# zifuwan/Sigma

Measured on AMD Instinct MI355X. Metric: images/sec fwd+bwd sigma_small 480x640, higher is better.
Workload: dtype f32

## Files before the change

include/sigma_ops.h:

```cpp
#ifndef SIGMA_OPS_H_
#define SIGMA_OPS_H_

#include <stdint.h>

#ifdef __cplusplus
extern "C" {
#endif

enum sigma_ops_status {
    SIGMA_OPS_OK = 0,
    SIGMA_OPS_ERR_ARG = 1,
    SIGMA_OPS_ERR_LAUNCH = 5
};

typedef struct sigma_dwconv_params {
    int32_t batch, channels, height, width;
    int32_t n_orders;
    int32_t flags;
    const float *x;
    const float *weight;
    const float *bias;
    float *out2;
    const float *g2;
    float *gpre;
// ... 14 lines not shown
typedef struct sigma_merge_params {
    int32_t batch, channels, height, width;
    const float *planes4;
    float *planes2;
    float *nhwc;
} sigma_merge_params;

int sigma_cross_merge_nhwc(const sigma_merge_params *params, void *stream);
int sigma_cross_split_nhwc(const sigma_merge_params *params, void *stream);

typedef struct sigma_transpose_params {
    int32_t batch, rows, cols, reserved_;
    const float *src;
    float *dst;
    int64_t src_batch_stride, src_row_stride, dst_batch_stride, dst_row_stride;
} sigma_transpose_params;

int sigma_transpose2d(const sigma_transpose_params *params, void *stream);

int sigma_pair_sum_add(const float *src, float *acc, int64_t n_outer, int64_t inner, void *stream);

int sigma_upsample2x_nhwc(const float *in, float *out, int32_t batch, int32_t height, int32_t width, int32_t channels,
                          int32_t backward, void *stream);

int sigma_plane_pool(const float *x, int64_t planes, int64_t hw, float *mean, float *max, float *count, void *stream);
int sigma_plane_scale(const float *x, const float *scale, float *out, int64_t planes, int64_t hw, void *stream);
int sigma_plane_dot(const float *a, const float *b, float *out, int64_t planes, int64_t hw, void *stream);
typedef struct sigma_gate_bwd_params {
    int64_t planes, hw;
    const float *g;
    const float *x;
    const float *scale;
    const float *dmean;
    const float *dmax;
    const float *max;
    const float *count;
    float *dx;
} sigma_gate_bwd_params;
int sigma_plane_gate_bwd(const sigma_gate_bwd_params *params, void *stream);

#define SIGMA_CE_BLOCKS 1024
int sigma_softmax_ce_fwd(const float *logits, const int64_t *labels, int64_t rows, int32_t classes, int64_t ignore_index,
                         float *lse, float *partial, void *stream);
int sigma_softmax_ce_bwd(const float *logits, const int64_t *labels, const float *lse, const float *scale, int64_t rows,
                         int32_t classes, int64_t ignore_index, float *dlogits, void *stream);
int sigma_softmax_ce_fwd_ld(const float *logits, const int64_t *labels, int64_t rows, int32_t classes, int32_t ld,
// ... 155 lines not shown
```

sigma_amd/_capi.py:

```python
from __future__ import annotations

import ctypes
import os
from typing import Optional

_HERE = os.path.dirname(os.path.abspath(__file__))
LIB_PATH = os.environ.get("SIGMA_HIP_LIB") or os.path.join(_HERE, "lib", "libsigma_hip.so")

SIGMA_SCAN_ABI_VERSION = 13
SIGMA_SCAN_CHUNK = 2048
SIGMA_SCAN_CKPT_PITCH = 1280
SIGMA_SCAN_CKPT_PITCH_FINE = 640
SIGMA_SCAN_CKPT_PITCH_320 = 320
SIGMA_SCAN_CKPT_PITCH_160 = 160
SIGMA_SCAN_CKPT_PITCH_16 = 16
SIGMA_SCAN_MAX_DSTATE = 256
SIGMA_SCAN_BWD_DETERMINISTIC = 1
SIGMA_DWCONV_DETERMINISTIC = 1

DTYPE_F32, DTYPE_F16, DTYPE_BF16 = 0, 1, 2


class SigmaHipUnavailable(RuntimeError):
    pass
# ... 60 lines not shown
class TransposeParams(ctypes.Structure):
    _fields_ = [
        ("batch", ctypes.c_int32), ("rows", ctypes.c_int32), ("cols", ctypes.c_int32), ("reserved_", ctypes.c_int32),
        ("src", ctypes.c_void_p), ("dst", ctypes.c_void_p),
        ("src_batch_stride", ctypes.c_int64), ("src_row_stride", ctypes.c_int64),
        ("dst_batch_stride", ctypes.c_int64), ("dst_row_stride", ctypes.c_int64),
    ]


class LayerNormParams(ctypes.Structure):
    _fields_ = [
        ("rows", ctypes.c_int64), ("channels", ctypes.c_int32), ("eps", ctypes.c_float),
        ("x", ctypes.c_void_p), ("gamma", ctypes.c_void_p), ("beta", ctypes.c_void_p),
        ("y", ctypes.c_void_p), ("mean", ctypes.c_void_p), ("rstd", ctypes.c_void_p),
        ("dy", ctypes.c_void_p), ("dx", ctypes.c_void_p), ("dgamma", ctypes.c_void_p), ("dbeta", ctypes.c_void_p),
        ("workspace", ctypes.c_void_p),
        ("gate", ctypes.c_void_p), ("gate_row_stride", ctypes.c_int64), ("dgate", ctypes.c_void_p),
        ("dgate_row_stride", ctypes.c_int64),
        ("row_scale", ctypes.c_void_p), ("rows_per_scale", ctypes.c_int64),
        ("dx_add", ctypes.c_void_p),
    ]


class GemmParams(ctypes.Structure):
    _fields_ = [
        ("M", ctypes.c_int64), ("N", ctypes.c_int32), ("K", ctypes.c_int32),
        ("A", ctypes.c_void_p), ("Bt", ctypes.c_void_p), ("C", ctypes.c_void_p), ("bias", ctypes.c_void_p),
        ("lda", ctypes.c_int64), ("ldb", ctypes.c_int64), ("ldc", ctypes.c_int64),
        ("accumulate", ctypes.c_int32), ("batch", ctypes.c_int32),
        ("strideA", ctypes.c_int64), ("strideB", ctypes.c_int64), ("strideC", ctypes.c_int64),
        ("a_mod", ctypes.c_int32), ("pieces", ctypes.c_int32),
        ("c_mod", ctypes.c_int32), ("reserved", ctypes.c_int32),
        ("residual", ctypes.c_void_p), ("residual2", ctypes.c_void_p), ("ldr", ctypes.c_int64), ("strideR", ctypes.c_int64),
        ("Ct", ctypes.c_void_p), ("ldct", ctypes.c_int64), ("t_cols", ctypes.c_int32), ("k_slices", ctypes.c_int32),
        ("workspace", ctypes.c_void_p), ("workspace_bytes", ctypes.c_int64),
    ]


class GateBwdParams(ctypes.Structure):
    _fields_ = [
        ("planes", ctypes.c_int64), ("hw", ctypes.c_int64),
        ("g", ctypes.c_void_p), ("x", ctypes.c_void_p), ("scale", ctypes.c_void_p), ("dmean", ctypes.c_void_p),
        ("dmax", ctypes.c_void_p), ("max", ctypes.c_void_p), ("count", ctypes.c_void_p), ("dx", ctypes.c_void_p),
    ]


# ... 47 lines not shown
    _fields_ = [
        ("batch", ctypes.c_int32), ("height", ctypes.c_int32), ("width", ctypes.c_int32), ("scale", ctypes.c_int32),
        ("classes", ctypes.c_int32), ("ld", ctypes.c_int32), ("ignore_index", ctypes.c_int64),
        ("kind", ctypes.c_int32), ("label_smoothing", ctypes.c_float), ("gamma", ctypes.c_float), ("reserved_", ctypes.c_int32),
        ("logits", ctypes.c_void_p), ("labels", ctypes.c_void_p), ("weight", ctypes.c_void_p), ("lse", ctypes.c_void_p),
        ("row_loss", ctypes.c_void_p), ("coef", ctypes.c_void_p), ("partial", ctypes.c_void_p),
        ("scale_grad", ctypes.c_void_p), ("row_grad", ctypes.c_void_p), ("dlogits", ctypes.c_void_p),
    ]


SIGMA_CE_BLOCKS = 1024
SIGMA_UPSAMPLE_LOSS_OPTIONS, SIGMA_UPSAMPLE_LOSS_FOCAL = 0, 1
SIGMA_OHEM_HIST_BLOCKS = 512
SIGMA_SEG_LDS_HIST_BYTES = 32768

GEMM_FORMS = {"nt": 0, "nn": 1, "tn": 2}
GEMM_EPILOGUES = ("rows", "direct", "transposed")
GEMM_RES_LOADS = ("none", "vector", "scalar")
GEMM_STORES = ("store", "accumulate", "atomic")

STRUCTS = {
    "sigma_scan_fwd_params": FwdParams, "sigma_scan_bwd_params": BwdParams,
    "sigma_dwconv_params": DwConvParams, "sigma_merge_params": MergeParams, "sigma_transpose_params": TransposeParams,
    "sigma_layernorm_params": LayerNormParams, "sigma_gate_bwd_params": GateBwdParams,
    "sigma_seg_accumulate_params": SegAccumulateParams, "sigma_seg_confusion_params": SegConfusionParams,
    "sigma_ce_opt_params": CeOptParams, "sigma_ohem_params": OhemParams, "sigma_upsample_ce_params": UpsampleCeParams,
    "sigma_upsample_loss_params": UpsampleLossParams,
    "sigma_gemm_params": GemmParams,
}

_I32, _I64, _INT, _F32, _VP, _STR = (ctypes.c_int32, ctypes.c_int64, ctypes.c_int, ctypes.c_float, ctypes.c_void_p,
                                     ctypes.c_char_p)
_P = ctypes.POINTER


def _params_stream(struct, *names):
    return {n: (_INT, [_P(struct), _VP]) for n in names}


_SCAN_SIGNATURES = {
    **_params_stream(FwdParams, "sigma_selective_scan_fwd"),
    **_params_stream(BwdParams, "sigma_selective_scan_bwd"),
    "sigma_scan_bwd_workspace_bytes": (_I64, [_P(BwdParams)]),
    "sigma_scan_fwd_workspace_bytes": (_I64, [_P(FwdParams)]),
    "sigma_scan_last_error": (_STR, []),
    "sigma_scan_abi_version": (_INT, []),
    "sigma_scan_set_option": (_INT, [_STR, _INT]),
    "sigma_scan_get_option": (_INT, [_STR]),
    "sigma_scan_fwd_plan": (_INT, [_P(FwdParams), _P(_I32 * 6)]),
    "sigma_scan_bwd_plan": (_INT, [_P(BwdParams), _P(_I32 * 6)]),
    "sigma_scan_selftest": (_INT, [_VP]),
    "sigma_scan_rowlane_selftest": (_INT, [_VP]),
}
_OPS_SIGNATURES = {
    **_params_stream(DwConvParams, "sigma_dwconv3x3_silu_fwd", "sigma_dwconv3x3_silu_bwd"),
    **_params_stream(MergeParams, "sigma_cross_merge_nhwc", "sigma_cross_split_nhwc"),
    **_params_stream(LayerNormParams, "sigma_layernorm_fwd", "sigma_layernorm_bwd"),
    "sigma_layernorm_bwd_partial_rows": (_INT, [_I64, _I32]),
    **_params_stream(TransposeParams, "sigma_transpose2d"),
    "sigma_pair_sum_add": (_INT, [_VP, _VP, _I64, _I64, _VP]),
    "sigma_upsample2x_nhwc": (_INT, [_VP, _VP, _I32, _I32, _I32, _I32, _I32, _VP]),
    "sigma_plane_pool": (_INT, [_VP, _I64, _I64, _VP, _VP, _VP, _VP]),
    "sigma_plane_scale": (_INT, [_VP, _VP, _VP, _I64, _I64, _VP]),
    "sigma_plane_dot": (_INT, [_VP, _VP, _VP, _I64, _I64, _VP]),
    **_params_stream(GateBwdParams, "sigma_plane_gate_bwd"),
    "sigma_softmax_ce_fwd": (_INT, [_VP, _VP, _I64, _I32, _I64, _VP, _VP, _VP]),
    "sigma_softmax_ce_bwd": (_INT, [_VP, _VP, _VP, _VP, _I64, _I32, _I64, _VP, _VP]),
    "sigma_softmax_ce_fwd_ld": (_INT, [_VP, _VP, _I64, _I32, _I32, _I64, _VP, _VP, _VP]),
    "sigma_softmax_ce_bwd_ld": (_INT, [_VP, _VP, _VP, _VP, _I64, _I32, _I32, _I64, _VP, _VP]),
    **_params_stream(CeOptParams, "sigma_softmax_ce_opt_fwd", "sigma_softmax_ce_opt_bwd"),
    "sigma_colscale_bwd": (_INT, [_VP, _VP, _VP, _VP, _VP, _I64, _I32, _VP]),
    "sigma_colscale_bwd_ws": (_INT, [_VP, _VP, _VP, _VP, _VP, _I64, _I32, _VP, _I64, _VP]),
    **_params_stream(SegAccumulateParams, "sigma_seg_accumulate"),
    **_params_stream(SegConfusionParams, "sigma_seg_argmax_confusion"),
    **_params_stream(OhemParams, "sigma_ohem_select"),
    "sigma_softmax_focal_fwd": (_INT, [_P(CeOptParams), _F32, _VP]),
    "sigma_softmax_focal_bwd": (_INT, [_P(CeOptParams), _F32, _VP]),
    **_params_stream(UpsampleCeParams, "sigma_upsample_ce_fwd", "sigma_upsample_ce_bwd"),
    **_params_stream(UpsampleLossParams, "sigma_upsample_loss_fwd", "sigma_upsample_loss_bwd"),
}
_OPS_AUX_SIGNATURES = {
    "sigma_dwconv3x3_silu_bwd_workspace_bytes": (_I64, [_P(DwConvParams)]),
    "sigma_colscale_bwd_workspace_bytes": (_I64, [_I64, _I32]),
    "sigma_ohem_workspace_bytes": (_I64, [_I64]),
# ... 70 lines not shown
```

sigma_amd/csrc/layernorm.hip:

```cpp
#include <hip/hip_runtime.h>
#include <stdint.h>

#include "../../include/sigma_ops.h"
#include "scan_device.h"

namespace sigma {

namespace {

__device__ __forceinline__ float wave_allsum(float v) { return wave_sum(v); }

struct LnArgs {
    const float* x; const float* gamma; const float* beta; const float* dy;
    float* y; float* mean; float* rstd; float* dx; float* ws;
    const float* z; float* dz; long z_stride, dz_stride;
    const float* rsc; long rows_per_scale;
    const float* dx_add;
    long M; int C; float eps;
};

__device__ __forceinline__ float sigmoid_f(float v) {
    return __builtin_amdgcn_rcpf(1.0f + __builtin_amdgcn_exp2f(-v * 1.4426950408889634f));
}

// ... 277 lines not shown
    return cached;
}

int fwd_grid(long rows, int C) {
    int occ = 8;
    dispatch_nv(C, [&](auto nv) { occ = resident_blocks<decltype(nv)::value, false>(); });
    return grid_blocks(rows, 256L * occ);
}

int bwd_grid(long rows, int C) {
    int occ = 8;
    dispatch_nv(C, [&](auto nv) { occ = resident_blocks<decltype(nv)::value, true>(); });
    long cap = bwd_blocks(rows, C);
    if (cap > 256L * occ) cap = 256L * occ;
    return grid_blocks(rows, cap);
}

bool check(const sigma_layernorm_params* p) {
    return p && p->rows >= 0 && p->channels > 0 && p->channels % 4 == 0 && p->channels <= 2048;
}

}

}

extern "C" {

int sigma_layernorm_bwd_partial_rows(int64_t rows, int32_t channels) {
    return sigma::bwd_grid(rows, channels > 0 ? channels : 4);
}

int sigma_layernorm_fwd(const sigma_layernorm_params* p, void* stream) {
    if (!sigma::check(p)) return SIGMA_OPS_ERR_ARG;
    if (p->rows == 0) return SIGMA_OPS_OK;
    if (!p->x || !p->gamma || !p->y) return SIGMA_OPS_ERR_ARG;
    sigma::LnArgs a{};
    a.x = p->x; a.gamma = p->gamma; a.beta = p->beta; a.y = p->y; a.mean = p->mean; a.rstd = p->rstd;
    a.z = p->gate; a.z_stride = p->gate_row_stride;
    if (p->gate && (p->gate_row_stride % 4 != 0 || p->gate_row_stride < p->channels)) return SIGMA_OPS_ERR_ARG;
    a.rsc = p->row_scale; a.rows_per_scale = p->rows_per_scale;
    if (p->row_scale && p->rows_per_scale <= 0) return SIGMA_OPS_ERR_ARG;
    a.M = p->rows; a.C = p->channels; a.eps = p->eps;
    const int grid = sigma::fwd_grid(p->rows, p->channels);
    hipStream_t s = static_cast<hipStream_t>(stream);
    const bool ok = sigma::dispatch_nv(p->channels, [&](auto nv) {
        hipLaunchKernelGGL(sigma::ln_fwd_kernel<decltype(nv)::value>, dim3(grid), dim3(256), 0, s, a);
// ... 38 lines not shown
```

sigma_amd/csrc/upsample.hip:

```cpp
#include <hip/hip_runtime.h>
#include <stdint.h>

#include "../../include/sigma_ops.h"

namespace sigma {
namespace {

struct Tap { int i0, i1; float w0, w1; };

__device__ __forceinline__ Tap tap_of(int dst, int n) {
    float src = (dst + 0.5f) * 0.5f - 0.5f;
    src = src < 0.0f ? 0.0f : src;
    Tap t;
    t.i0 = (int)src;
    t.i1 = t.i0 + 1 < n ? t.i0 + 1 : n - 1;
    t.w1 = src - (float)t.i0;
    t.w0 = 1.0f - t.w1;
    return t;
}

__device__ __forceinline__ float weight_of(int o, int i, int n) {
    const Tap t = tap_of(o, n);
    return (t.i0 == i ? t.w0 : 0.0f) + (t.i1 == i ? t.w1 : 0.0f);
}

__global__ void __launch_bounds__(256)
// ... 34 lines not shown
            const int oy = 2 * y - 1 + k, ox = 2 * x - 1 + k;
            wy[k] = (oy >= 0 && oy < OH) ? weight_of(oy, y, H) : 0.0f;
            wx[k] = (ox >= 0 && ox < OW) ? weight_of(ox, x, W) : 0.0f;
        }
        const float4* __restrict__ base = g + (long)b * OH * OW * C4 + c;
        float4 acc = make_float4(0.f, 0.f, 0.f, 0.f);
#pragma unroll
        for (int ky = 0; ky < 4; ++ky) {
            int oy = 2 * y - 1 + ky;
            oy = oy < 0 ? 0 : (oy >= OH ? OH - 1 : oy);
#pragma unroll
            for (int kx = 0; kx < 4; ++kx) {
                int ox = 2 * x - 1 + kx;
                ox = ox < 0 ? 0 : (ox >= OW ? OW - 1 : ox);
                const float w = wy[ky] * wx[kx];
                const float4 v = base[((long)oy * OW + ox) * C4];
                acc.x = fmaf(w, v.x, acc.x); acc.y = fmaf(w, v.y, acc.y); acc.z = fmaf(w, v.z, acc.z); acc.w = fmaf(w, v.w, acc.w);
            }
        }
        din[idx] = acc;
    }
}

}
}

extern "C" int sigma_upsample2x_nhwc(const float* in, float* out, int32_t batch, int32_t height, int32_t width, int32_t channels,
                                     int32_t backward, void* stream) {
    if (!in || !out || batch < 0 || height <= 0 || width <= 0 || channels <= 0 || channels % 4 != 0) return SIGMA_OPS_ERR_ARG;
    if ((reinterpret_cast<uintptr_t>(in) | reinterpret_cast<uintptr_t>(out)) & 15u) return SIGMA_OPS_ERR_ARG;
    if (batch == 0) return SIGMA_OPS_OK;
    const int C4 = channels / 4;
    const long work = backward ? (long)batch * height * width * C4 : (long)batch * 4 * height * width * C4;
    long blocks = (work + 255) / 256;
    if (blocks > 256L * 64) blocks = 256L * 64;
    hipStream_t s = static_cast<hipStream_t>(stream);
    if (backward)
        hipLaunchKernelGGL(sigma::up2x_bwd_kernel, dim3((unsigned)blocks), dim3(256), 0, s, reinterpret_cast<const float4*>(in),
                           reinterpret_cast<float4*>(out), batch, height, width, C4);
    else
        hipLaunchKernelGGL(sigma::up2x_fwd_kernel, dim3((unsigned)blocks), dim3(256), 0, s, reinterpret_cast<const float4*>(in),
                           reinterpret_cast<float4*>(out), batch, height, width, C4);
    return hipGetLastError() == hipSuccess ? SIGMA_OPS_OK : SIGMA_OPS_ERR_LAUNCH;
}
```

sigma_amd/layernorm.py:

```python
from __future__ import annotations

import ctypes

import torch
import torch.nn as nn
import torch.nn.functional as F

from . import _capi
from ._handoff import offer_xz_grad_buffer
from ._launch import launch


def _gate_view(z: torch.Tensor, C: int):
    if z.stride(-1) == 1 and z.dim() >= 2:
        zs = z.reshape(-1, C) if z.is_contiguous() else None
        if zs is not None:
            return zs, C
        st = z.stride(-2)
        ok = all(z.stride(i) == z.stride(i + 1) * z.shape[i + 1] for i in range(z.dim() - 2))
        if ok and st % 4 == 0 and st >= C and z.data_ptr() % 16 == 0:
            return z, st
    zc = z.contiguous()
    return zc, C

# ... 80 lines not shown
            p.dgate_row_stride = 2 * C
        else:
            dz = torch.empty(ctx.gate_shape, device=xc.device, dtype=torch.float32)
        p.beta = bias.data_ptr() if ctx.has_bias else None
        p.gate, p.gate_row_stride, p.dgate = zk.data_ptr(), ctx.zstride, dz.data_ptr()
    launch("sigma_layernorm_bwd", ctypes.byref(p), device=xc.device, what="layernorm_bwd")
    return dx, dgamma, dbeta, None, dz, None


class LayerNormResidualFn(torch.autograd.Function):

    @staticmethod
    def forward(ctx, x, weight, bias, eps):
        y = LayerNormFn.forward(ctx, x, weight, bias, eps)
        return y, x.view_as(x)

    @staticmethod
    def backward(ctx, dy, dpass):
        if dy is None:
            return dpass, None, None, None
        return _ln_backward(ctx, dy, dpass)[:4]


def _aligned16(*tensors) -> bool:
    return all(t is None or (t.data_ptr() % 16 == 0 and t.is_cuda and t.dtype == torch.float32) for t in tensors)


class LayerNorm(nn.LayerNorm):

    def forward(self, x: torch.Tensor) -> torch.Tensor:
        C = x.shape[-1] if x.dim() > 0 else 0
        if (x.is_cuda and x.dtype == torch.float32 and self.elementwise_affine and len(self.normalized_shape) == 1
                and C % 4 == 0 and 0 < C <= 2048 and x.numel() > 0
                and _aligned16(self.weight, self.bias) and (not x.is_contiguous() or x.data_ptr() % 16 == 0)):
            return LayerNormFn.apply(x, self.weight, self.bias, self.eps)
        return F.layer_norm(x, self.normalized_shape, self.weight, self.bias, self.eps)

    def forward_with_pass(self, x: torch.Tensor):
        C = x.shape[-1] if x.dim() > 0 else 0
        if (x.is_cuda and x.dtype == torch.float32 and self.elementwise_affine and len(self.normalized_shape) == 1
                and C % 4 == 0 and 0 < C <= 2048 and x.numel() > 0 and x.requires_grad and torch.is_grad_enabled()
                and _aligned16(self.weight, self.bias) and x.is_contiguous() and x.data_ptr() % 16 == 0):
            return LayerNormResidualFn.apply(x, self.weight, self.bias, self.eps)
        return self.forward(x), x

    def forward_gated(self, x: torch.Tensor, z: torch.Tensor, row_scale=None) -> torch.Tensor:
        C = x.shape[-1]
        if (x.is_cuda and x.dtype == torch.float32 and z.dtype == torch.float32 and self.elementwise_affine
                and len(self.normalized_shape) == 1 and C % 4 == 0 and 0 < C <= 2048 and x.numel() > 0
                and tuple(z.shape) == tuple(x.shape) and _aligned16(self.weight, self.bias)
                and (not x.is_contiguous() or x.data_ptr() % 16 == 0)):
            return LayerNormFn.apply(x, self.weight, self.bias, self.eps, z, row_scale)
        y = self.forward(x) * F.silu(z)
        return y if row_scale is None else y * row_scale.reshape(-1, *([1] * (y.dim() - 1)))
```

sigma_amd/models/decoders/MambaDecoder.py:

```python
from __future__ import annotations

import torch
import torch.nn as nn

from ..._launch import launch, ptr
from ...layernorm import LayerNorm
import torch.nn.functional as F

from ..encoders.vmamba import CVSSDecoderBlock


class _Up2xFn(torch.autograd.Function):

    @staticmethod
    def forward(ctx, x):
        B, H, W, C = x.shape
        out = torch.empty(B, 2 * H, 2 * W, C, device=x.device, dtype=torch.float32)
        launch("sigma_upsample2x_nhwc", ptr(x), ptr(out), B, H, W, C, 0, device=x.device, what="upsample2x_nhwc")
        ctx.dims = (B, H, W, C)
        return out

    @staticmethod
    def backward(ctx, g):
        B, H, W, C = ctx.dims
        g = g.contiguous()
        dx = torch.empty(B, H, W, C, device=g.device, dtype=torch.float32)
        launch("sigma_upsample2x_nhwc", ptr(g), ptr(dx), B, H, W, C, 1, device=g.device, what="upsample2x_nhwc (adjoint)")
        return dx


def _up2(x_nhwc: torch.Tensor) -> torch.Tensor:
    if x_nhwc.is_cuda and x_nhwc.dtype == torch.float32 and x_nhwc.shape[-1] % 4 == 0 and x_nhwc.numel() > 0:
        return _Up2xFn.apply(x_nhwc.contiguous())
    y = F.interpolate(x_nhwc.permute(0, 3, 1, 2), scale_factor=2, mode="bilinear", align_corners=False)
    return y.permute(0, 2, 3, 1)


_INTERP = {}


def interp_matrix(n: int, s: int, device, dtype=torch.float32) -> torch.Tensor:
    key = (int(n), int(s), torch.device(device), dtype)
    U = _INTERP.get(key)
    if U is None:
        num = (2 * torch.arange(n * s, device=device) + 1 - s).clamp_min(0)
        i0 = torch.div(num, 2 * s, rounding_mode="floor")
        lam = ((num - i0 * 2 * s).to(dtype) / (2 * s))[:, None]
        i1 = (i0 + 1).clamp_max(n - 1)
        col = torch.arange(n, device=device)[None, :]
        U = (col == i0[:, None]).to(dtype) * (1 - lam) + (col == i1[:, None]).to(dtype) * lam
        if not (U.is_cuda and torch.cuda.is_current_stream_capturing()) and not torch.is_inference_mode_enabled():
            _INTERP[key] = U
    return U


def expand_logits(z: torch.Tensor, s: int) -> torch.Tensor:
    B, h, w, nc = z.shape
    ld = (nc + 3) // 4 * 4 if z.is_cuda else nc
# ... 13 lines not shown
        self.dim = dim
        self.expand = nn.Linear(dim, 2 * dim, bias=False) if dim_scale == 2 else nn.Identity()
        self.norm = norm_layer(dim // dim_scale)

    def forward(self, x):
        x = self.expand(x)
        B, H, W, C = x.shape
        x = x.view(B, H, W, 2, 2, C // 4).permute(0, 1, 3, 2, 4, 5).reshape(B, 2 * H, 2 * W, C // 4)
        return self.norm(x)


class UpsampleExpand(nn.Module):

    def __init__(self, input_resolution, dim, patch_size=4, norm_layer=LayerNorm):
        super().__init__()
        self.input_resolution = input_resolution
        self.dim = dim
        self.patch_size = patch_size
        self.linear = nn.Linear(dim, dim // 2, bias=False)
        self.output_dim = dim
        self.norm = norm_layer(dim // 2)

    def forward(self, x):
        return self.norm(_up2(self.linear(x)))


class FinalUpsample_X4(nn.Module):

    def __init__(self, input_resolution, dim, patch_size=4, norm_layer=LayerNorm):
        super().__init__()
        self.input_resolution = input_resolution
        self.dim = dim
        self.patch_size = patch_size
        self.linear1 = nn.Linear(dim, dim, bias=False)
        self.linear2 = nn.Linear(dim, dim, bias=False)
        self.output_dim = dim
        self.norm = norm_layer(dim)

    def forward(self, x):
        x = _up2(self.linear1(x))
        x = _up2(self.linear2(x))
        return self.norm(x)


class Mamba_up(nn.Module):

    def __init__(self, dim, input_resolution, depth, dt_rank="auto", d_state=4, ssm_ratio=2.0, attn_drop_rate=0.0,
                 drop_rate=0.0, mlp_ratio=4.0, drop_path=0.1, norm_layer=LayerNorm, upsample=None,
                 use_checkpoint=False, **kwargs):
        super().__init__()
        self.input_resolution = input_resolution
        self.depth = depth
        rates = drop_path if isinstance(drop_path, (list, tuple)) else [drop_path] * depth
        self.blocks = nn.ModuleList([
            CVSSDecoderBlock(hidden_dim=dim, drop_path=rates[i], norm_layer=norm_layer, attn_drop_rate=attn_drop_rate,
                             d_state=d_state, dt_rank=dt_rank, ssm_ratio=ssm_ratio) for i in range(depth)])
        self.upsample = (UpsampleExpand(input_resolution, dim=dim, patch_size=2, norm_layer=norm_layer)
                         if upsample is not None else None)

    def forward(self, x):
        for blk in self.blocks:
            x = blk(x)
        return x if self.upsample is None else self.upsample(x)


# ... 81 lines not shown
```

Baseline: 50.69.

## Fuse bilinear 2x upsample with LayerNorm in decoder forward and backward

Adds fused HIP kernels that compute the 2x bilinear upsample and the following LayerNorm in one pass, so the 4x-larger upsampled tensor is never written and re-read. The forward kernel processes cells of four output pixels sharing four input taps, with software prefetch of the next cell. The backward kernel strips the image, folds the upsample adjoint into the LayerNorm gradient through shared-memory exchange between neighbouring cells, and reduces dgamma/dbeta through a workspace. It adds a lot of complex kernel code and constrains channel counts to 96/192/384.

Result: no change. 51.07, median of 6 (+0.8%).

```diff
diff --git a/include/sigma_ops.h b/include/sigma_ops.h
--- a/include/sigma_ops.h
+++ b/include/sigma_ops.h
@@ -60,6 +60,27 @@
 
 int sigma_upsample2x_nhwc(const float *in, float *out, int32_t batch, int32_t height, int32_t width, int32_t channels,
                           int32_t backward, void *stream);
+
+typedef struct sigma_upsample_ln_params {
+    int32_t batch, height, width, channels;
+    float eps;
+    int32_t reserved_;
+    const float *t;
+    const float *gamma;
+    const float *beta;
+    float *y;
+    float *mean;
+    float *rstd;
+    const float *dy;
+    float *dt;
+    float *dgamma;
+    float *dbeta;
+    float *workspace;
+} sigma_upsample_ln_params;
+
+int sigma_upsample2x_ln_fwd(const sigma_upsample_ln_params *params, void *stream);
+int sigma_upsample2x_ln_bwd(const sigma_upsample_ln_params *params, void *stream);
+int sigma_upsample2x_ln_bwd_partial_rows(int32_t batch, int32_t height, int32_t width, int32_t channels);
 
 int sigma_plane_pool(const float *x, int64_t planes, int64_t hw, float *mean, float *max, float *count, void *stream);
 int sigma_plane_scale(const float *x, const float *scale, float *out, int64_t planes, int64_t hw, void *stream);
diff --git a/sigma_amd/_capi.py b/sigma_amd/_capi.py
--- a/sigma_amd/_capi.py
+++ b/sigma_amd/_capi.py
@@ -106,6 +106,17 @@
     ]
 
 
+class UpsampleLnParams(ctypes.Structure):
+    _fields_ = [
+        ("batch", ctypes.c_int32), ("height", ctypes.c_int32), ("width", ctypes.c_int32), ("channels", ctypes.c_int32),
+        ("eps", ctypes.c_float), ("reserved_", ctypes.c_int32),
+        ("t", ctypes.c_void_p), ("gamma", ctypes.c_void_p), ("beta", ctypes.c_void_p),
+        ("y", ctypes.c_void_p), ("mean", ctypes.c_void_p), ("rstd", ctypes.c_void_p),
+        ("dy", ctypes.c_void_p), ("dt", ctypes.c_void_p), ("dgamma", ctypes.c_void_p), ("dbeta", ctypes.c_void_p),
+        ("workspace", ctypes.c_void_p),
+    ]
+
+
 class GemmParams(ctypes.Structure):
     _fields_ = [
         ("M", ctypes.c_int64), ("N", ctypes.c_int32), ("K", ctypes.c_int32),
@@ -199,7 +210,8 @@
 STRUCTS = {
     "sigma_scan_fwd_params": FwdParams, "sigma_scan_bwd_params": BwdParams,
     "sigma_dwconv_params": DwConvParams, "sigma_merge_params": MergeParams, "sigma_transpose_params": TransposeParams,
-    "sigma_layernorm_params": LayerNormParams, "sigma_gate_bwd_params": GateBwdParams,
+    "sigma_layernorm_params": LayerNormParams, "sigma_upsample_ln_params": UpsampleLnParams,
+    "sigma_gate_bwd_params": GateBwdParams,
     "sigma_seg_accumulate_params": SegAccumulateParams, "sigma_seg_confusion_params": SegConfusionParams,
     "sigma_ce_opt_params": CeOptParams, "sigma_ohem_params": OhemParams, "sigma_upsample_ce_params": UpsampleCeParams,
     "sigma_upsample_loss_params": UpsampleLossParams,
@@ -237,6 +249,8 @@
     **_params_stream(TransposeParams, "sigma_transpose2d"),
     "sigma_pair_sum_add": (_INT, [_VP, _VP, _I64, _I64, _VP]),
     "sigma_upsample2x_nhwc": (_INT, [_VP, _VP, _I32, _I32, _I32, _I32, _I32, _VP]),
+    **_params_stream(UpsampleLnParams, "sigma_upsample2x_ln_fwd", "sigma_upsample2x_ln_bwd"),
+    "sigma_upsample2x_ln_bwd_partial_rows": (_INT, [_I32, _I32, _I32, _I32]),
     "sigma_plane_pool": (_INT, [_VP, _I64, _I64, _VP, _VP, _VP, _VP]),
     "sigma_plane_scale": (_INT, [_VP, _VP, _VP, _I64, _I64, _VP]),
     "sigma_plane_dot": (_INT, [_VP, _VP, _VP, _I64, _I64, _VP]),
diff --git a/sigma_amd/csrc/layernorm.hip b/sigma_amd/csrc/layernorm.hip
--- a/sigma_amd/csrc/layernorm.hip
+++ b/sigma_amd/csrc/layernorm.hip
@@ -323,6 +323,11 @@
 
 }
 
+int ln_reduce_launch(const float* ws, float* dgamma, float* dbeta, int nrows, int C, hipStream_t s) {
+    hipLaunchKernelGGL(ln_reduce_kernel, dim3((2 * C + 15) / 16), dim3(256), 0, s, ws, dgamma, dbeta, nrows, C);
+    return hipGetLastError() == hipSuccess ? SIGMA_OPS_OK : SIGMA_OPS_ERR_LAUNCH;
+}
+
 }
 
 extern "C" {
diff --git a/sigma_amd/csrc/upsample.hip b/sigma_amd/csrc/upsample.hip
--- a/sigma_amd/csrc/upsample.hip
+++ b/sigma_amd/csrc/upsample.hip
@@ -1,7 +1,10 @@
 #include <hip/hip_runtime.h>
 #include <stdint.h>
 
+#include <type_traits>
+
 #include "../../include/sigma_ops.h"
+#include "scan_device.h"
 
 namespace sigma {
 namespace {
@@ -82,7 +85,394 @@
     }
 }
 
-}
+template <int C> struct UpLnMap {
+    static_assert(C == 96 || C == 192 || C == 384, "channel counts of the decoder");
+    static constexpr int LPP = C == 96 ? 32 : 64;
+    static constexpr int NV = (C + 255) / 256;
+    static constexpr int GPB = 256 / LPP;
+    static constexpr int CPG = C == 384 ? 1 : 2;
+};
+
+struct UpLnArgs {
+    const float* t; const float* gamma; const float* beta; const float* dy; const float* mean_in; const float* rstd_in;
+    float* y; float* mean; float* rstd; float* dt; float* ws;
+    int B, H, W; float eps;
+    int nstrip, nseg, seg_h;
+};
+
+template <int LPP>
+__device__ __forceinline__ float group_sum(float v) {
+    if constexpr (LPP == 64) {
+        return wave_sum(v);
+    } else {
+        v += dpp_take<DPP_ROW_SHR1, 0xF>(0.0f, v);
+        v += dpp_take<DPP_ROW_SHR2, 0xF>(0.0f, v);
+        v += dpp_take<DPP_ROW_SHR4, 0xF>(0.0f, v);
+        v += dpp_take<DPP_ROW_SHR8, 0xF>(0.0f, v);
+        v += dpp_take<DPP_ROW_BCAST15, 0xA>(0.0f, v);
+        const float lo = __builtin_bit_cast(float, __builtin_amdgcn_readlane(__builtin_bit_cast(int, v), 31));
+        const float hi = __builtin_bit_cast(float, __builtin_amdgcn_readlane(__builtin_bit_cast(int, v), 63));
+        return (threadIdx.x & 32) ? hi : lo;
+    }
+}
+
+__device__ __forceinline__ float4 lerp4(const Tap& ty, const Tap& tx, const float4& a, const float4& b, const float4& c, const float4& d) {
+    float4 o;
+    o.x = ty.w0 * (tx.w0 * a.x + tx.w1 * b.x) + ty.w1 * (tx.w0 * c.x + tx.w1 * d.x);
+    o.y = ty.w0 * (tx.w0 * a.y + tx.w1 * b.y) + ty.w1 * (tx.w0 * c.y + tx.w1 * d.y);
+    o.z = ty.w0 * (tx.w0 * a.z + tx.w1 * b.z) + ty.w1 * (tx.w0 * c.z + tx.w1 * d.z);
+    o.w = ty.w0 * (tx.w0 * a.w + tx.w1 * b.w) + ty.w1 * (tx.w0 * c.w + tx.w1 * d.w);
+    return o;
+}
+
+struct CellAxis { bool v[2]; int f[2]; Tap t[2]; };
+__device__ __forceinline__ CellAxis cell_axis(int cb, int n) {
+    CellAxis a;
+    a.v[0] = cb >= 1; a.v[1] = cb < n;
+    a.f[0] = a.v[0] ? 2 * cb - 1 : 0;
+    a.f[1] = a.v[1] ? 2 * cb : 2 * n - 1;
+    a.t[0] = tap_of(a.f[0], n); a.t[1] = tap_of(a.f[1], n);
+    return a;
+}
+
+__device__ __forceinline__ float tap_weight(const Tap& t, int i) {
+    return (t.i0 == i ? t.w0 : 0.0f) + (t.i1 == i ? t.w1 : 0.0f);
+}
+
+template <int C>
+__global__ void __launch_bounds__(256) up2x_ln_fwd_kernel(const UpLnArgs a) {
+    using M = UpLnMap<C>;
+    constexpr int LPP = M::LPP, NV = M::NV, GPB = M::GPB;
+    const int l = threadIdx.x & (LPP - 1);
+    const int H = a.H, W = a.W, OH = 2 * H, OW = 2 * W;
+    const int per_img = (H + 1) * (W + 1);
+    const int ncells = a.B * per_img;
+    const int ngrp = gridDim.x * GPB;
+    int coff[NV];
+    bool live[NV];
+    float4 g[NV], bt[NV];
+#pragma unroll
+    for (int j = 0; j < NV; ++j) {
+        const int c = l * 4 + 256 * j;
+        live[j] = c < C;
+        coff[j] = live[j] ? c : 0;
+        g[j] = *reinterpret_cast<const float4*>(a.gamma + coff[j]);
+        bt[j] = *reinterpret_cast<const float4*>(a.beta + coff[j]);
+    }
+    const float inv = 1.0f / (float)C;
+    auto load_cell = [&](int cell, float4 (&q)[4][NV]) {
+        const int b = cell / per_img, r = cell - b * per_img, yb = r / (W + 1), xb = r - yb * (W + 1);
+        const Tap ty = tap_of(yb >= 1 ? 2 * yb - 1 : 0, H), tx = tap_of(xb >= 1 ? 2 * xb - 1 : 0, W);
+        const float* __restrict__ base = a.t + (long)b * H * W * C;
+#pragma unroll
+        for (int j = 0; j < NV; ++j) {
+            q[0][j] = *reinterpret_cast<const float4*>(base + ((long)ty.i0 * W + tx.i0) * C + coff[j]);
+            q[1][j] = *reinterpret_cast<const float4*>(base + ((long)ty.i0 * W + tx.i1) * C + coff[j]);
+            q[2][j] = *reinterpret_cast<const float4*>(base + ((long)ty.i1 * W + tx.i0) * C + coff[j]);
+            q[3][j] = *reinterpret_cast<const float4*>(base + ((long)ty.i1 * W + tx.i1) * C + coff[j]);
+        }
+    };
+    const int first = blockIdx.x * GPB + threadIdx.x / LPP;
+    float4 cur[4][NV];
+    load_cell(first < ncells ? first : ncells - 1, cur);
+    for (int base = blockIdx.x * GPB; base < ncells; base += ngrp) {
+        const int want = base + threadIdx.x / LPP;
+        const bool cell_ok = want < ncells;
+        const int cell = cell_ok ? want : ncells - 1;
+        float4 nxt[4][NV];
+        const bool more = base + ngrp < ncells;
+        if (more) load_cell(want + ngrp < ncells ? want + ngrp : ncells - 1, nxt);
+        const int b = cell / per_img, r = cell - b * per_img, yb = r / (W + 1), xb = r - yb * (W + 1);
+        const CellAxis ay = cell_axis(yb, H), ax = cell_axis(xb, W);
+        float4 v[4][NV];
+        float s[4];
+#pragma unroll
+        for (int p = 0; p < 4; ++p) {
+            s[p] = 0.0f;
+#pragma unroll
+            for (int j = 0; j < NV; ++j) {
+                v[p][j] = lerp4(ay.t[p >> 1], ax.t[p & 1], cur[0][j], cur[1][j], cur[2][j], cur[3][j]);
+                if (live[j]) s[p] += (v[p][j].x + v[p][j].y) + (v[p][j].z + v[p][j].w);
+            }
+        }
+        float mu[4], rs[4];
+#pragma unroll
+        for (int p = 0; p < 4; ++p) mu[p] = group_sum<LPP>(s[p]) * inv;
+#pragma unroll
+        for (int p = 0; p < 4; ++p) {
+            float q = 0.0f;
+#pragma unroll
+            for (int j = 0; j < NV; ++j) {
+                if (live[j]) {
+                    const float d0 = v[p][j].x - mu[p], d1 = v[p][j].y - mu[p], d2 = v[p][j].z - mu[p], d3 = v[p][j].w - mu[p];
+                    q += (d0 * d0 + d1 * d1) + (d2 * d2 + d3 * d3);
+                }
+            }
+            s[p] = q;
+        }
+#pragma unroll
+        for (int p = 0; p < 4; ++p) rs[p] = rsqrtf(group_sum<LPP>(s[p]) * inv + a.eps);
+#pragma unroll
+        for (int p = 0; p < 4; ++p) {
+            if (!(cell_ok && ay.v[p >> 1] && ax.v[p & 1])) continue;
+            const long pix = ((long)b * OH + ay.f[p >> 1]) * OW + ax.f[p & 1];
+            float* __restrict__ yr = a.y + pix * C;
+#pragma unroll
+            for (int j = 0; j < NV; ++j) {
+                if (live[j]) {
+                    float4 o;
+                    o.x = (v[p][j].x - mu[p]) * rs[p] * g[j].x + bt[j].x;
+                    o.y = (v[p][j].y - mu[p]) * rs[p] * g[j].y + bt[j].y;
+                    o.z = (v[p][j].z - mu[p]) * rs[p] * g[j].z + bt[j].z;
+                    o.w = (v[p][j].w - mu[p]) * rs[p] * g[j].w + bt[j].w;
+                    *reinterpret_cast<float4*>(yr + coff[j]) = o;
+                }
+            }
+            if (l == 0 && a.mean) { a.mean[pix] = mu[p]; a.rstd[pix] = rs[p]; }
+        }
+        if (more) {
+#pragma unroll
+            for (int p = 0; p < 4; ++p)
+#pragma unroll
+                for (int j = 0; j < NV; ++j) cur[p][j] = nxt[p][j];
+        }
+    }
+}
+
+template <int C>
+__global__ void __launch_bounds__(256) up2x_ln_bwd_kernel(const UpLnArgs a) {
+    using M = UpLnMap<C>;
+    constexpr int LPP = M::LPP, NV = M::NV, GPB = M::GPB, CPG = M::CPG, NCELL = GPB * CPG, SW = NCELL - 1;
+    static_assert(GPB * 2 * C <= 2 * NCELL * C, "the partial rows reuse the exchange buffers");
+    __shared__ float xch[2 * NCELL * C];
+    const int l = threadIdx.x & (LPP - 1), grp = threadIdx.x / LPP;
+    const int H = a.H, W = a.W, OH = 2 * H, OW = 2 * W;
+    const int strip = blockIdx.x % a.nstrip, seg = (blockIdx.x / a.nstrip) % a.nseg, b = blockIdx.x / (a.nstrip * a.nseg);
+    const int x0 = strip * SW, x1 = x0 + SW < W ? x0 + SW : W;
+    const int y0 = seg * a.seg_h, y1 = y0 + a.seg_h < H ? y0 + a.seg_h : H;
+    int coff[NV];
+    bool live[NV];
+    float4 gam[NV], dg[NV], db[NV];
+#pragma unroll
+    for (int j = 0; j < NV; ++j) {
+        const int c = l * 4 + 256 * j;
+        live[j] = c < C;
+        coff[j] = live[j] ? c : 0;
+        gam[j] = *reinterpret_cast<const float4*>(a.gamma + coff[j]);
+        dg[j] = make_float4(0, 0, 0, 0);
+        db[j] = make_float4(0, 0, 0, 0);
+    }
+    const float inv = 1.0f / (float)C;
+    const float* __restrict__ tb = a.t + (long)b * H * W * C;
+    bool act[CPG], ownx[CPG];
+    int xbs[CPG];
+    CellAxis ax[CPG];
+    float wxl[CPG][2], wxr[CPG][2];
+    float4 carl[CPG][NV], carr[CPG][NV];
+#pragma unroll
+    for (int k = 0; k < CPG; ++k) {
+        const int xb = x0 + grp * CPG + k;
+        act[k] = xb <= x1;
+        xbs[k] = xb;
+        ownx[k] = act[k] && (xb < x1 || x1 == W);
+        ax[k] = cell_axis(act[k] ? xb : x1, W);
+#pragma unroll
+        for (int c = 0; c < 2; ++c) {
+            const bool ok = act[k] && ax[k].v[c];
+            wxl[k][c] = (ok && xb >= 1) ? tap_weight(ax[k].t[c], xb - 1) : 0.0f;
+            wxr[k][c] = (ok && xb < W) ? tap_weight(ax[k].t[c], xb) : 0.0f;
+        }
+#pragma unroll
+        for (int j = 0; j < NV; ++j) { carl[k][j] = make_float4(0, 0, 0, 0); carr[k][j] = make_float4(0, 0, 0, 0); }
+    }
+    for (int yb = y0; yb <= y1; ++yb) {
+        float* __restrict__ xb_buf = xch + ((yb - y0) & 1) * (NCELL * C);
+        const CellAxis ay = cell_axis(yb, H);
+        const bool owny = yb < y1 || y1 == H;
+        float wyu[2], wyl[2];
+#pragma unroll
+        for (int r = 0; r < 2; ++r) {
+            wyu[r] = (ay.v[r] && yb >= 1) ? tap_weight(ay.t[r], yb - 1) : 0.0f;
+            wyl[r] = (ay.v[r] && yb < H) ? tap_weight(ay.t[r], yb) : 0.0f;
+        }
+        float4 q[CPG][4][NV], gy[CPG][4][NV];
+        float mu[CPG][4], rs[CPG][4];
+#pragma unroll
+        for (int k = 0; k < CPG; ++k) {
+            const Tap& ty = ay.t[0];
+            const Tap& tx = ax[k].t[0];
+#pragma unroll
+            for (int j = 0; j < NV; ++j) {
+                q[k][0][j] = *reinterpret_cast<const float4*>(tb + ((long)ty.i0 * W + tx.i0) * C + coff[j]);
+                q[k][1][j] = *reinterpret_cast<const float4*>(tb + ((long)ty.i0 * W + tx.i1) * C + coff[j]);
+                q[k][2][j] = *reinterpret_cast<const float4*>(tb + ((long)ty.i1 * W + tx.i0) * C + coff[j]);
+                q[k][3][j] = *reinterpret_cast<const float4*>(tb + ((long)ty.i1 * W + tx.i1) * C + coff[j]);
+            }
+#pragma unroll
+            for (int p = 0; p < 4; ++p) {
+                const long pix = ((long)b * OH + ay.f[p >> 1]) * OW + ax[k].f[p & 1];
+                mu[k][p] = a.mean_in[pix];
+                rs[k][p] = a.rstd_in[pix];
+#pragma unroll
+                for (int j = 0; j < NV; ++j) gy[k][p][j] = *reinterpret_cast<const float4*>(a.dy + pix * C + coff[j]);
+            }
+        }
+        float4 xh[CPG][4][NV], tt[CPG][4][NV];
+        float s1[CPG][4], s2[CPG][4];
+#pragma unroll
+        for (int k = 0; k < CPG; ++k) {
+#pragma unroll
+            for (int p = 0; p < 4; ++p) {
+                const bool valid = act[k] && ay.v[p >> 1] && ax[k].v[p & 1];
+                const float om = (valid && ownx[k] && owny) ? 1.0f : 0.0f;
+                s1[k][p] = 0.0f;
+                s2[k][p] = 0.0f;
+#pragma unroll
+                for (int j = 0; j < NV; ++j) {
+                    const float4 v = lerp4(ay.t[p >> 1], ax[k].t[p & 1], q[k][0][j], q[k][1][j], q[k][2][j], q[k][3][j]);
+                    float4 gv = gy[k][p][j];
+                    if (!(valid && live[j])) gv = make_float4(0, 0, 0, 0);
+                    const float4 h = make_float4((v.x - mu[k][p]) * rs[k][p], (v.y - mu[k][p]) * rs[k][p], (v.z - mu[k][p]) * rs[k][p],
+                                                 (v.w - mu[k][p]) * rs[k][p]);
+                    const float4 t = make_float4(gv.x * gam[j].x, gv.y * gam[j].y, gv.z * gam[j].z, gv.w * gam[j].w);
+                    s1[k][p] += (t.x + t.y) + (t.z + t.w);
+                    s2[k][p] += (t.x * h.x + t.y * h.y) + (t.z * h.z + t.w * h.w);
+                    dg[j].x += (gv.x * om) * h.x; dg[j].y += (gv.y * om) * h.y; dg[j].z += (gv.z * om) * h.z; dg[j].w += (gv.w * om) * h.w;
+                    db[j].x += gv.x * om; db[j].y += gv.y * om; db[j].z += gv.z * om; db[j].w += gv.w * om;
+                    xh[k][p][j] = h;
+                    tt[k][p][j] = t;
+                }
+            }
+        }
+#pragma unroll
+        for (int k = 0; k < CPG; ++k) {
+#pragma unroll
+            for (int p = 0; p < 4; ++p) {
+                s1[k][p] = group_sum<LPP>(s1[k][p]) * inv;
+                s2[k][p] = group_sum<LPP>(s2[k][p]) * inv;
+            }
+        }
+        float4 totr[CPG][NV];
+#pragma unroll
+        for (int k = 0; k < CPG; ++k) {
+#pragma unroll
+            for (int j = 0; j < NV; ++j) {
+                float4 hl[2], hr[2];
+#pragma unroll
+                for (int r = 0; r < 2; ++r) {
+                    float4 dx[2];
+#pragma unroll
+                    for (int c = 0; c < 2; ++c) {
+                        const int p = 2 * r + c;
+                        const float4 t = tt[k][p][j], h = xh[k][p][j];
+                        const float m1 = s1[k][p], m2 = s2[k][p], rsp = rs[k][p];
+                        dx[c] = make_float4(rsp * (t.x - m1 - h.x * m2), rsp * (t.y - m1 - h.y * m2), rsp * (t.z - m1 - h.z * m2),
+                                            rsp * (t.w - m1 - h.w * m2));
+                    }
+                    hl[r] = make_float4(wxl[k][0] * dx[0].x + wxl[k][1] * dx[1].x, wxl[k][0] * dx[0].y + wxl[k][1] * dx[1].y,
+                                        wxl[k][0] * dx[0].z + wxl[k][1] * dx[1].z, wxl[k][0] * dx[0].w + wxl[k][1] * dx[1].w);
+                    hr[r] = make_float4(wxr[k][0] * dx[0].x + wxr[k][1] * dx[1].x, wxr[k][0] * dx[0].y + wxr[k][1] * dx[1].y,
+                                        wxr[k][0] * dx[0].z + wxr[k][1] * dx[1].z, wxr[k][0] * dx[0].w + wxr[k][1] * dx[1].w);
+                }
+                const float4 ul = make_float4(wyu[0] * hl[0].x + wyu[1] * hl[1].x, wyu[0] * hl[0].y + wyu[1] * hl[1].y,
+                                              wyu[0] * hl[0].z + wyu[1] * hl[1].z, wyu[0] * hl[0].w + wyu[1] * hl[1].w);
+                const float4 ur = make_float4(wyu[0] * hr[0].x + wyu[1] * hr[1].x, wyu[0] * hr[0].y + wyu[1] * hr[1].y,
+                                              wyu[0] * hr[0].z + wyu[1] * hr[1].z, wyu[0] * hr[0].w + wyu[1] * hr[1].w);
+                const float4 totl = make_float4(carl[k][j].x + ul.x, carl[k][j].y + ul.y, carl[k][j].z + ul.z, carl[k][j].w + ul.w);
+                totr[k][j] = make_float4(carr[k][j].x + ur.x, carr[k][j].y + ur.y, carr[k][j].z + ur.z, carr[k][j].w + ur.w);
+                carl[k][j] = make_float4(wyl[0] * hl[0].x + wyl[1] * hl[1].x, wyl[0] * hl[0].y + wyl[1] * hl[1].y,
+                                         wyl[0] * hl[0].z + wyl[1] * hl[1].z, wyl[0] * hl[0].w + wyl[1] * hl[1].w);
+                carr[k][j] = make_float4(wyl[0] * hr[0].x + wyl[1] * hr[1].x, wyl[0] * hr[0].y + wyl[1] * hr[1].y,
+                                         wyl[0] * hr[0].z + wyl[1] * hr[1].z, wyl[0] * hr[0].w + wyl[1] * hr[1].w);
+                if (live[j]) *reinterpret_cast<float4*>(xb_buf + (grp * CPG + k) * C + coff[j]) = totl;
+            }
+        }
+        __syncthreads();
+        if (yb > y0) {
+#pragma unroll
+            for (int k = 0; k < CPG; ++k) {
+                if (act[k] && xbs[k] < x1) {
+                    float* __restrict__ dr = a.dt + (((long)b * H + (yb - 1)) * W + xbs[k]) * C;
+#pragma unroll
+                    for (int j = 0; j < NV; ++j) {
+                        if (live[j]) {
+                            const float4 nb = *reinterpret_cast<const float4*>(xb_buf + (grp * CPG + k + 1) * C + coff[j]);
+                            *reinterpret_cast<float4*>(dr + coff[j]) =
+                                make_float4(totr[k][j].x + nb.x, totr[k][j].y + nb.y, totr[k][j].z + nb.z, totr[k][j].w + nb.w);
+                        }
+                    }
+                }
+            }
+        }
+    }
+    __syncthreads();
+    float* __restrict__ part = xch;
+#pragma unroll
+    for (int j = 0; j < NV; ++j) {
+        if (live[j]) {
+            *reinterpret_cast<float4*>(part + (grp * 2 + 0) * C + coff[j]) = dg[j];
+            *reinterpret_cast<float4*>(part + (grp * 2 + 1) * C + coff[j]) = db[j];
+        }
+    }
+    __syncthreads();
+    float* __restrict__ wrow = a.ws + (long)blockIdx.x * 2 * C;
+    for (int i = threadIdx.x; i < 2 * C; i += 256) {
+        float acc = part[i];
+#pragma unroll
+        for (int gq = 1; gq < GPB; ++gq) acc += part[gq * 2 * C + i];
+        wrow[i] = acc;
+    }
+}
+
+struct UpLnPlan { int nstrip, seg_h, nseg; long grid; };
+
+template <typename F>
+bool dispatch_c(int C, F&& f) {
+    switch (C) {
+        case 96: f(std::integral_constant<int, 96>()); return true;
+        case 192: f(std::integral_constant<int, 192>()); return true;
+        case 384: f(std::integral_constant<int, 384>()); return true;
+        default: return false;
+    }
+}
+
+bool upln_sizes_ok(int B, int H, int W, int C) {
+    if (B < 0 || H <= 0 || W <= 0 || !(C == 96 || C == 192 || C == 384)) return false;
+    const long cells = (long)(B > 0 ? B : 1) * (H + 1) * (W + 1), fine = 4L * (B > 0 ? B : 1) * H * W;
+    return cells < (1L << 31) && fine < (1L << 31);
+}
+
+UpLnPlan plan_bwd(int B, int H, int W, int C) {
+    UpLnPlan p{};
+    int sw = 1;
+    dispatch_c(C, [&](auto c) { using M = UpLnMap<decltype(c)::value>; sw = M::GPB * M::CPG - 1; });
+    p.nstrip = (W + sw - 1) / sw;
+    long sh = ((long)B * H * p.nstrip + 2047) / 2048;
+    if (sh < 8) sh = 8;
+    if (sh > H) sh = H;
+    p.seg_h = (int)sh;
+    p.nseg = (H + p.seg_h - 1) / p.seg_h;
+    p.grid = (long)B * p.nseg * p.nstrip;
+    return p;
+}
+
+template <int C>
+int fwd_resident_blocks() {
+    static int cached = 0;
+    if (cached == 0) {
+        int n = 0;
+        const hipError_t e = hipOccupancyMaxActiveBlocksPerMultiprocessor(&n, up2x_ln_fwd_kernel<C>, 256, 0);
+        cached = (e == hipSuccess && n > 0) ? (n > 8 ? 8 : n) : 4;
+    }
+    return cached;
+}
+
+bool aligned16(const void* p) { return (reinterpret_cast<uintptr_t>(p) & 15u) == 0; }
+
+}
+
+int ln_reduce_launch(const float* ws, float* dgamma, float* dbeta, int nrows, int C, hipStream_t s);
+
 }
 
 extern "C" int sigma_upsample2x_nhwc(const float* in, float* out, int32_t batch, int32_t height, int32_t width, int32_t channels,
@@ -103,3 +493,57 @@
                            reinterpret_cast<float4*>(out), batch, height, width, C4);
     return hipGetLastError() == hipSuccess ? SIGMA_OPS_OK : SIGMA_OPS_ERR_LAUNCH;
 }
+
+extern "C" int sigma_upsample2x_ln_bwd_partial_rows(int32_t batch, int32_t height, int32_t width, int32_t channels) {
+    if (!sigma::upln_sizes_ok(batch, height, width, channels)) return -1;
+    if (batch == 0) return 0;
+    return (int)sigma::plan_bwd(batch, height, width, channels).grid;
+}
+
+extern "C" int sigma_upsample2x_ln_fwd(const sigma_upsample_ln_params* p, void* stream) {
+    if (!p || !sigma::upln_sizes_ok(p->batch, p->height, p->width, p->channels)) return SIGMA_OPS_ERR_ARG;
+    if (!p->t || !p->gamma || !p->beta || !p->y || (p->mean == nullptr) != (p->rstd == nullptr)) return SIGMA_OPS_ERR_ARG;
+    if (!sigma::aligned16(p->t) || !sigma::aligned16(p->gamma) || !sigma::aligned16(p->beta) || !sigma::aligned16(p->y))
+        return SIGMA_OPS_ERR_ARG;
+    if ((reinterpret_cast<uintptr_t>(p->mean) | reinterpret_cast<uintptr_t>(p->rstd)) & 3u) return SIGMA_OPS_ERR_ARG;
+    if (p->batch == 0) return SIGMA_OPS_OK;
+    sigma::UpLnArgs a{};
+    a.t = p->t; a.gamma = p->gamma; a.beta = p->beta; a.y = p->y; a.mean = p->mean; a.rstd = p->rstd;
+    a.B = p->batch; a.H = p->height; a.W = p->width; a.eps = p->eps;
+    const long cells = (long)p->batch * (p->height + 1) * (p->width + 1);
+    hipStream_t s = static_cast<hipStream_t>(stream);
+    sigma::dispatch_c(p->channels, [&](auto c) {
+        constexpr int C = decltype(c)::value;
+        constexpr int GPB = sigma::UpLnMap<C>::GPB;
+        long blocks = (cells + GPB - 1) / GPB;
+        const long cap = 256L * sigma::fwd_resident_blocks<C>();
+        if (blocks > cap) blocks = cap;
+        hipLaunchKernelGGL(sigma::up2x_ln_fwd_kernel<C>, dim3((unsigned)blocks), dim3(256), 0, s, a);
+    });
+    return hipGetLastError() == hipSuccess ? SIGMA_OPS_OK : SIGMA_OPS_ERR_LAUNCH;
+}
+
+extern "C" int sigma_upsample2x_ln_bwd(const sigma_upsample_ln_params* p, void* stream) {
+    if (!p || !sigma::upln_sizes_ok(p->batch, p->height, p->width, p->channels)) return SIGMA_OPS_ERR_ARG;
+    if (!p->dgamma || !p->dbeta) return SIGMA_OPS_ERR_ARG;
+    hipStream_t s = static_cast<hipStream_t>(stream);
+    if (p->batch == 0) return sigma::ln_reduce_launch(p->workspace, p->dgamma, p->dbeta, 0, p->channels, s);
+    if (!p->t || !p->gamma || !p->dy || !p->mean || !p->rstd || !p->dt || !p->workspace) return SIGMA_OPS_ERR_ARG;
+    if (!sigma::aligned16(p->t) || !sigma::aligned16(p->gamma) || !sigma::aligned16(p->dy) || !sigma::aligned16(p->dt) ||
+        !sigma::aligned16(p->workspace))
+        return SIGMA_OPS_ERR_ARG;
+    if ((reinterpret_cast<uintptr_t>(p->mean) | reinterpret_cast<uintptr_t>(p->rstd) | reinterpret_cast<uintptr_t>(p->dgamma) |
+         reinterpret_cast<uintptr_t>(p->dbeta)) & 3u)
+        return SIGMA_OPS_ERR_ARG;
+    const sigma::UpLnPlan pl = sigma::plan_bwd(p->batch, p->height, p->width, p->channels);
+    if (pl.grid > 0x7fffffffL) return SIGMA_OPS_ERR_ARG;
+    sigma::UpLnArgs a{};
+    a.t = p->t; a.gamma = p->gamma; a.dy = p->dy; a.mean_in = p->mean; a.rstd_in = p->rstd; a.dt = p->dt; a.ws = p->workspace;
+    a.B = p->batch; a.H = p->height; a.W = p->width; a.eps = p->eps;
+    a.nstrip = pl.nstrip; a.nseg = pl.nseg; a.seg_h = pl.seg_h;
+    sigma::dispatch_c(p->channels, [&](auto c) {
+        hipLaunchKernelGGL(sigma::up2x_ln_bwd_kernel<decltype(c)::value>, dim3((unsigned)pl.grid), dim3(256), 0, s, a);
+    });
+    if (hipGetLastError() != hipSuccess) return SIGMA_OPS_ERR_LAUNCH;
+    return sigma::ln_reduce_launch(p->workspace, p->dgamma, p->dbeta, (int)pl.grid, p->channels, s);
+}
diff --git a/sigma_amd/layernorm.py b/sigma_amd/layernorm.py
--- a/sigma_amd/layernorm.py
+++ b/sigma_amd/layernorm.py
@@ -126,6 +126,50 @@
         return _ln_backward(ctx, dy, dpass)[:4]
 
 
+UPSAMPLE_LN_CHANNELS = (96, 192, 384)
+
+
+class Upsample2xLayerNormFn(torch.autograd.Function):
+
+    @staticmethod
+    def forward(ctx, t, weight, bias, eps):
+        B, H, W, C = t.shape
+        y = torch.empty(B, 2 * H, 2 * W, C, device=t.device, dtype=torch.float32)
+        need_bwd = any(ctx.needs_input_grad)
+        mean = torch.empty(B * 4 * H * W, device=t.device, dtype=torch.float32) if need_bwd else None
+        rstd = torch.empty_like(mean) if need_bwd else None
+        p = _capi.UpsampleLnParams()
+        p.batch, p.height, p.width, p.channels, p.eps = B, H, W, C, float(eps)
+        p.t, p.gamma, p.beta, p.y = t.data_ptr(), weight.data_ptr(), bias.data_ptr(), y.data_ptr()
+        if need_bwd:
+            p.mean, p.rstd = mean.data_ptr(), rstd.data_ptr()
+        launch("sigma_upsample2x_ln_fwd", ctypes.byref(p), device=t.device, what="upsample2x_ln_fwd")
+        if need_bwd:
+            ctx.save_for_backward(t, weight, mean, rstd)
+            ctx.eps = float(eps)
+        return y
+
+    @staticmethod
+    def backward(ctx, dy):
+        t, weight, mean, rstd = ctx.saved_tensors
+        B, H, W, C = t.shape
+        dy = dy.contiguous()
+        if dy.data_ptr() % 16:
+            dy = dy.clone()
+        dt = torch.empty_like(t)
+        dgamma, dbeta = torch.empty_like(weight), torch.empty_like(weight)
+        nrows = int(_capi.load().sigma_upsample2x_ln_bwd_partial_rows(B, H, W, C))
+        if nrows < 0:
+            raise RuntimeError(f"upsample2x_ln_bwd: sizes ({B}, {H}, {W}, {C}) are refused")
+        ws = torch.empty(max(nrows, 1) * 2 * C, device=t.device, dtype=torch.float32)
+        p = _capi.UpsampleLnParams()
+        p.batch, p.height, p.width, p.channels, p.eps = B, H, W, C, ctx.eps
+        p.t, p.gamma, p.mean, p.rstd = t.data_ptr(), weight.data_ptr(), mean.data_ptr(), rstd.data_ptr()
+        p.dy, p.dt, p.dgamma, p.dbeta, p.workspace = dy.data_ptr(), dt.data_ptr(), dgamma.data_ptr(), dbeta.data_ptr(), ws.data_ptr()
+        launch("sigma_upsample2x_ln_bwd", ctypes.byref(p), device=t.device, what="upsample2x_ln_bwd")
+        return dt, dgamma, dbeta, None
+
+
 def _aligned16(*tensors) -> bool:
     return all(t is None or (t.data_ptr() % 16 == 0 and t.is_cuda and t.dtype == torch.float32) for t in tensors)
 
@@ -147,6 +191,16 @@
                 and _aligned16(self.weight, self.bias) and x.is_contiguous() and x.data_ptr() % 16 == 0):
             return LayerNormResidualFn.apply(x, self.weight, self.bias, self.eps)
         return self.forward(x), x
+
+    def forward_upsampled(self, t: torch.Tensor):
+        if (type(self) is LayerNorm and self.elementwise_affine and self.bias is not None and len(self.normalized_shape) == 1
+                and t.dim() == 4 and t.is_cuda and t.dtype == torch.float32 and t.is_contiguous() and t.numel() > 0
+                and t.shape[-1] in UPSAMPLE_LN_CHANNELS and self.normalized_shape[0] == t.shape[-1]
+                and 4 * t.shape[0] * t.shape[1] * t.shape[2] < 2 ** 31 and t.data_ptr() % 16 == 0
+                and _aligned16(self.weight, self.bias)
+                and not (self._forward_hooks or self._forward_pre_hooks or self._backward_hooks or self._backward_pre_hooks)):
+            return Upsample2xLayerNormFn.apply(t, self.weight, self.bias, self.eps)
+        return None
 
     def forward_gated(self, x: torch.Tensor, z: torch.Tensor, row_scale=None) -> torch.Tensor:
         C = x.shape[-1]
diff --git a/sigma_amd/models/decoders/MambaDecoder.py b/sigma_amd/models/decoders/MambaDecoder.py
--- a/sigma_amd/models/decoders/MambaDecoder.py
+++ b/sigma_amd/models/decoders/MambaDecoder.py
@@ -34,6 +34,14 @@
         return _Up2xFn.apply(x_nhwc.contiguous())
     y = F.interpolate(x_nhwc.permute(0, 3, 1, 2), scale_factor=2, mode="bilinear", align_corners=False)
     return y.permute(0, 2, 3, 1)
+
+
+def _up2_norm(x_nhwc: torch.Tensor, norm: nn.Module) -> torch.Tensor:
+    if type(norm) is LayerNorm:
+        y = norm.forward_upsampled(x_nhwc)
+        if y is not None:
+            return y
+    return norm(_up2(x_nhwc))
 
 
 _INTERP = {}
@@ -93,7 +101,7 @@
         self.norm = norm_layer(dim // 2)
 
     def forward(self, x):
-        return self.norm(_up2(self.linear(x)))
+        return _up2_norm(self.linear(x), self.norm)
 
 
 class FinalUpsample_X4(nn.Module):
@@ -110,8 +118,7 @@
 
     def forward(self, x):
         x = _up2(self.linear1(x))
-        x = _up2(self.linear2(x))
-        return self.norm(x)
+        return _up2_norm(self.linear2(x), self.norm)
 
 
 class Mamba_up(nn.Module):
```
